# NilsJochem/audio-matcher

Hardware: AMD Instinct MI355X
Metric: audio samples/s matched (whole node), 10 s needle vs 1 h haystack, 1/2/4/8 GPU (higher is better)
Workload: dtype f32

## Files before the change

audio-matcher_amd/build.py:

```python
from __future__ import annotations

import os
import shutil
import subprocess
import sys
from concurrent.futures import ThreadPoolExecutor

HERE = os.path.dirname(os.path.abspath(__file__))
CSRC = os.path.join(HERE, "csrc")
OBJ = os.path.join(HERE, "build")
LIB = os.path.join(HERE, "libaudiomatch_amd.so")
SOURCES = ["am_fft.hip", "am_peaks.hip", "am_context.hip", "am_correlate.hip", "am_engine.hip", "am_stream.hip", "am_monitor.hip", "am_pool.hip", "am_norm.hip", "am_hits.hip", "am_segments.hip", "am_bands.hip", "am_significance.hip", "am_resample.hip", "am_whiten.hip", "am_estimate.hip", "am_warp.hip", "am_channel.hip", "am_stereo.hip",
           "am_best.hip", "am_trace.hip", "am_api.hip"]
HEADERS = [os.path.join(CSRC, "am_kernels.h"), os.path.join(CSRC, "am_internal.h"), os.path.join(CSRC, "am_walk.h"), os.path.join(CSRC, "am_spans.h"),
           os.path.join(HERE, "..", "include", "audiomatch.h")]
ARCH = "gfx950"
FLAGS = ["-O3", "-std=c++17", "-fPIC", f"--offload-arch={ARCH}", "-ffp-contract=fast", "-fno-slp-vectorize",
         "-Wall", "-Wno-unused-result"]


def _hipcc() -> str:
    for cand in (shutil.which("hipcc"), "/opt/rocm/bin/hipcc"):
        if cand and os.path.exists(cand):
            return cand
    raise RuntimeError("hipcc not found: the HIP extension cannot be built")


def _stale(target: str, deps: list[str]) -> bool:
    if not os.path.exists(target):
        return True
    t = os.path.getmtime(target)
    return any(os.path.getmtime(d) > t for d in deps if os.path.exists(d))


def build_library(force: bool = False, verbose: bool = False) -> str:
    srcs = [os.path.join(CSRC, s) for s in SOURCES]
    if not force and not _stale(LIB, srcs + HEADERS + [os.path.abspath(__file__)]):
# ... 82 lines not shown
```

audio-matcher_amd/csrc/am_fft.hip:

```cpp
#include "am_kernels.h"

#include <float.h>
#include <stdlib.h>
#include <algorithm>
#include <atomic>
#include <hip/hip_fp16.h>

namespace am {

__device__ __forceinline__ float2 cadd(float2 a, float2 b) { return make_float2(a.x + b.x, a.y + b.y); }
__device__ __forceinline__ float2 csub(float2 a, float2 b) { return make_float2(a.x - b.x, a.y - b.y); }
__device__ __forceinline__ float2 cmul(float2 a, float2 b) {
    return make_float2(a.x * b.x - a.y * b.y, a.x * b.y + a.y * b.x);
}
__device__ __forceinline__ float2 cmulc(float2 a, float2 b) {
    return make_float2(a.x * b.x + a.y * b.y, a.y * b.x - a.x * b.y);
}
__device__ __forceinline__ float2 mul_neg_i(float2 a) { return make_float2(a.y, -a.x); }
__device__ __forceinline__ float2 mul_pos_i(float2 a) { return make_float2(-a.y, a.x); }

__device__ __forceinline__ float2 tw_big(const PlanDev& pl, unsigned m) {
    return cmul(pl.twhi[m >> pl.logLo], pl.twlo[m & ((1u << pl.logLo) - 1u)]);
}

__device__ __forceinline__ void tw_big_pair(const PlanDev& pl, unsigned m, float2& w, float2& w4) {
    const float4 h = pl.twhi4[m >> pl.logLo], l = pl.twlo4[m & ((1u << pl.logLo) - 1u)];
    w = cmul(make_float2(h.x, h.y), make_float2(l.x, l.y));
    w4 = cmul(make_float2(h.z, h.w), make_float2(l.z, l.w));
}

__device__ constexpr float kCos32[16] = {
    1.0f, 0.9807852804032304f, 0.9238795325112867f, 0.8314696123025452f, 0.7071067811865476f,
    0.5555702330196023f, 0.38268343236508984f, 0.19509032201612833f, 0.0f, -0.1950903220161282f,
    -0.3826834323650897f, -0.555570233019602f, -0.7071067811865475f, -0.8314696123025453f,
    -0.9238795325112867f, -0.9807852804032304f};
__device__ constexpr float kSin32[16] = {
    0.0f, 0.19509032201612825f, 0.3826834323650898f, 0.5555702330196022f, 0.7071067811865475f,
    0.8314696123025452f, 0.9238795325112867f, 0.9807852804032304f, 1.0f, 0.9807852804032304f,
    0.9238795325112867f, 0.8314696123025455f, 0.7071067811865476f, 0.5555702330196022f,
    0.3826834323650899f, 0.1950903220161286f};

template <int R>
__host__ __device__ constexpr int brev(int i) {
    int r = 0;
    for (int b = 1; b < R; b <<= 1) { r = (r << 1) | (i & 1); i >>= 1; }
    return r;
}

template <bool INV>
__device__ __forceinline__ float2 mul_w32(float2 d, int idx) {
    if (idx == 0) return d;
    if (idx == 8) return INV ? mul_pos_i(d) : mul_neg_i(d);
    const float c = kCos32[idx], s = kSin32[idx];
    if (INV) return make_float2(d.x * c - d.y * s, d.x * s + d.y * c);
    return make_float2(d.x * c + d.y * s, d.y * c - d.x * s);
}

typedef _Float16 h2 __attribute__((ext_vector_type(2)));
__device__ __forceinline__ h2 cadd(h2 a, h2 b) { return a + b; }
__device__ __forceinline__ h2 csub(h2 a, h2 b) { return a - b; }
__device__ __forceinline__ h2 cmul(h2 a, h2 b) {
    const h2 t = a * b.xx;
    return __builtin_elementwise_fma(a.yx, (h2){-b.y, b.y}, t);
}
__device__ __forceinline__ h2 mul_neg_i(h2 a) { return (h2){a.y, -a.x}; }
__device__ __forceinline__ h2 mul_pos_i(h2 a) { return (h2){-a.y, a.x}; }
__device__ __forceinline__ h2 to_h2(float2 v) { return (h2){(_Float16)v.x, (_Float16)v.y}; }
__device__ __forceinline__ float2 to_f2(h2 v) { return make_float2((float)v.x, (float)v.y); }
__device__ __forceinline__ unsigned h2_bits(h2 v) { return __builtin_bit_cast(unsigned, v); }
__device__ __forceinline__ h2 bits_h2(unsigned u) { return __builtin_bit_cast(h2, u); }
template <bool INV>
__device__ __forceinline__ h2 mul_w32(h2 d, int idx) {
    if (idx == 0) return d;
    if (idx == 8) return INV ? mul_pos_i(d) : mul_neg_i(d);
    const _Float16 c = (_Float16)kCos32[idx], s = (_Float16)kSin32[idx];
    const h2 t = d * (h2){c, c};
    if (INV) return __builtin_elementwise_fma(d.yx, (h2){-s, s}, t);
    return __builtin_elementwise_fma(d.yx, (h2){s, -s}, t);
}

__device__ __forceinline__ float2 add_signed(float2 u, float2 v, float sgn) {
    return make_float2(fmaf(sgn, v.x, u.x), fmaf(sgn, v.y, u.y));
}

template <int R, bool INV, typename T>
__device__ __forceinline__ void dif(T* x) {
    if constexpr (R >= 2) {
#pragma unroll
        for (int i = 0; i < R / 2; ++i) {
            const T a = x[i], b = x[i + R / 2];
            x[i] = cadd(a, b);
            x[i + R / 2] = mul_w32<INV>(csub(a, b), i * (32 / R));
        }
        dif<R / 2, INV>(x);
        dif<R / 2, INV>(x + R / 2);
    }
}

template <int R, bool CONJ, bool BREV>
__device__ __forceinline__ void twiddle_apply(float2* x, float2 w) {
    float2 pw[R / 2 + 1];
    if (CONJ) w.y = -w.y;
    pw[1] = w;
    x[BREV ? brev<R>(1) : 1] = cmul(x[BREV ? brev<R>(1) : 1], w);
#pragma unroll
    for (int e = 2; e < R; ++e) {
        const float2 v = cmul(pw[(e + 1) / 2], pw[e / 2]);
        if (e <= R / 2) pw[e] = v;
        x[BREV ? brev<R>(e) : e] = cmul(x[BREV ? brev<R>(e) : e], v);
    }
}
template <int R, bool CONJ, bool BREV>
__device__ __forceinline__ void twiddle_apply(h2* x, float2 w) {
    float2 pw[R / 2 + 1];
    if (CONJ) w.y = -w.y;
    pw[1] = w;
    x[BREV ? brev<R>(1) : 1] = cmul(x[BREV ? brev<R>(1) : 1], to_h2(w));
#pragma unroll
    for (int e = 2; e < R; ++e) {
// ... 180 lines not shown
template <int KIND>
__device__ __forceinline__ void k1_load(const Job& job, long long col, int in_stride, int hi, long long baseA, long long baseB,
                                        bool validB, bool fast, float2 (&x0)[16], float2 (&x1)[16]) {
    if (fast) {
#pragma unroll
        for (int a = 0; a < 16; ++a) {
            const long long off = (long long)(a * 16 + hi) * in_stride + col;
            const float2 va = load_sample2<KIND>(job.src, baseA + off), vb = load_sample2<KIND>(job.src, baseB + off);
            x0[a] = make_float2(va.x, vb.x);
            x1[a] = make_float2(va.y, vb.y);
        }
    } else {
#pragma unroll
        for (int a = 0; a < 16; ++a) {
            const long long n = (long long)(a * 16 + hi) * in_stride + col;
            const float2 va = load2_padded<KIND>(job.src, baseA + n, job.src_len);
            const float2 vb = validB ? load2_padded<KIND>(job.src, baseB + n, job.src_len) : make_float2(0.f, 0.f);
            x0[a] = make_float2(va.x, vb.x);
            x1[a] = make_float2(va.y, vb.y);
        }
    }
}
__device__ __forceinline__ void k1_transform(const K1Twiddles& w, float2* lds2, int hi, int cp, float2 (&x0)[16], float2 (&x1)[16]) {
    dif<16, false>(x0);
    dif<16, false>(x1);
    twiddle_brev<16, false>(x0, w.w256, w.w256q);
    twiddle_brev<16, false>(x1, w.w256, w.w256q);
#pragma unroll
    for (int ap = 0; ap < 16; ++ap) lds2[(ap * 16 + hi) * 17 + cp] = x0[brev<16>(ap)];
    __syncthreads();
#pragma unroll
    for (int b = 0; b < 16; ++b) x0[b] = lds2[(hi * 16 + b) * 17 + cp];
    __syncthreads();
#pragma unroll
    for (int ap = 0; ap < 16; ++ap) lds2[(ap * 16 + hi) * 17 + cp] = x1[brev<16>(ap)];
    __syncthreads();
#pragma unroll
    for (int b = 0; b < 16; ++b) x1[b] = lds2[(hi * 16 + b) * 17 + cp];
    dif<16, false>(x0);
    dif<16, false>(x1);
    twiddle_chain<16, false, true>(x0, w.base0, w.step0, w.step0q);
    twiddle_chain<16, false, true>(x1, w.base1, w.step1, w.step1q);
}
template <int KIND>
__device__ __forceinline__ void k1_tile(const Job& job, const PlanDev& pl, float2* lds2, long long col, int in_stride,
                                        int hi, int cp, long long baseA, long long baseB, bool validB, bool fast,
                                        float2 (&x0)[16], float2 (&x1)[16]) {
    const K1Twiddles w = k1_twiddles(pl, col, hi);
    k1_load<KIND>(job, col, in_stride, hi, baseA, baseB, validB, fast, x0, x1);
    k1_transform(w, lds2, hi, cp, x0, x1);
}

__device__ __forceinline__ void k1_transform_h16(const K1Twiddles& w, uint2* ldsu, int hi, int cp, h2 (&x0)[16], h2 (&x1)[16]) {
    dif<16, false>(x0);
    dif<16, false>(x1);
    twiddle_apply2<16, false, true>(x0, x1, w.w256);
#pragma unroll
    for (int ap = 0; ap < 16; ++ap) ldsu[(ap * 16 + hi) * 17 + cp] = make_uint2(h2_bits(x0[brev<16>(ap)]), h2_bits(x1[brev<16>(ap)]));
    __syncthreads();
#pragma unroll
    for (int b = 0; b < 16; ++b) {
        const uint2 v = ldsu[(hi * 16 + b) * 17 + cp];
        x0[b] = bits_h2(v.x);
// ... 81 lines not shown
    float2 qj0, qj1, qc0, qc1;
};
__device__ __forceinline__ K2Lane k2_lane(const PlanDev& pl, int t = threadIdx.x) {
    K2Lane k;
    k.t = t; k.hi = k.t >> 4; k.cp = k.t & 15;
    k.voff = (unsigned)k.t * 16u;
    const float4 j = pl.k2j[2 * k.t], jq = pl.k2j[2 * k.t + 1], c = pl.k2c[2 * k.cp], cq = pl.k2c[2 * k.cp + 1];
    k.wj0 = make_float2(j.x, j.y); k.wj1 = make_float2(j.z, j.w);
    k.qj0 = make_float2(jq.x, jq.y); k.qj1 = make_float2(jq.z, jq.w);
    k.wc0 = make_float2(c.x, c.y); k.wc1 = make_float2(c.z, c.w);
    k.qc0 = make_float2(cq.x, cq.y); k.qc1 = make_float2(cq.z, cq.w);
    return k;
}

__device__ __forceinline__ void k2_forward12(const K2Lane& k, __amdgpu_buffer_rsrc_t rrow, float4* lds4) {
    const int t = k.t, hi = k.hi, cp = k.cp;
    float2 x0[16], x1[16];
#pragma unroll
    for (int a = 0; a < 16; ++a) {
        const float4 v = buf_load4(rrow, k.voff, a * 4096);
        x0[a] = make_float2(v.x, v.y);
        x1[a] = make_float2(v.z, v.w);
    }
    dif<16, false>(x0);
    dif<16, false>(x1);
    twiddle_brev<16, false>(x0, k.wj0, k.qj0);
    twiddle_brev<16, false>(x1, k.wj1, k.qj1);
#pragma unroll
    for (int ap = 0; ap < 16; ++ap)
        lds4[ap * 256 + t] = make_float4(x0[brev<16>(ap)].x, x0[brev<16>(ap)].y,
                                         x1[brev<16>(ap)].x, x1[brev<16>(ap)].y);
    __syncthreads();
#pragma unroll
    for (int b = 0; b < 16; ++b) {
        const float4 v = lds4[hi * 256 + b * 16 + cp];
        x0[b] = make_float2(v.x, v.y);
        x1[b] = make_float2(v.z, v.w);
    }
    dif<16, false>(x0);
    dif<16, false>(x1);
    twiddle_brev<16, false>(x0, k.wc0, k.qc0);
    twiddle_brev<16, false>(x1, k.wc1, k.qc1);
    wave_sync_lds();
#pragma unroll
    for (int bp = 0; bp < 16; ++bp)
        lds4[(hi * 16 + bp) * 16 + (cp ^ bp)] = make_float4(x0[brev<16>(bp)].x, x0[brev<16>(bp)].y,
                                                            x1[brev<16>(bp)].x, x1[brev<16>(bp)].y);
    wave_sync_lds();
}

__device__ __forceinline__ void k2_forward3(const K2Lane& k, const float4* lds4, float2 (&z)[32]) {
#pragma unroll
    for (int i = 0; i < 16; ++i) {
        const float4 v = lds4[k.t * 16 + (i ^ k.cp)];
        z[2 * i] = make_float2(v.x, v.y);
        z[2 * i + 1] = make_float2(v.z, v.w);
    }
    dif<32, false>(z);
}

__device__ __forceinline__ void k2_fetch_quarter(__amdgpu_buffer_rsrc_t rh, unsigned voff, int part, float4 (&h)[4]) {
#pragma unroll
    for (int i = 0; i < 4; ++i) h[i] = buf_load4(rh, voff, (part * 4 + i) * 4096);
}
__device__ __forceinline__ void k2_multiply_quarter(const float2 (&z)[32], const float4 (&h)[4], int part, float2 (&q)[32]) {
#pragma unroll
    for (int i = 0; i < 4; ++i) {
        const int e = part * 4 + i;
        q[brev<32>(2 * e)] = cmul(z[2 * e], make_float2(h[i].x, h[i].y));
        q[brev<32>(2 * e + 1)] = cmul(z[2 * e + 1], make_float2(h[i].z, h[i].w));
    }
}
__device__ __forceinline__ void k2_multiply_fetch(const float2 (&z)[32], __amdgpu_buffer_rsrc_t rh, unsigned voff,
                                                  const float4 (&first)[4], float2 (&q)[32]) {
    float4 ha[4], hb[4];
    k2_fetch_quarter(rh, voff, 1, ha);
    __builtin_amdgcn_sched_barrier(0);
    k2_multiply_quarter(z, first, 0, q);
    k2_fetch_quarter(rh, voff, 2, hb);
    __builtin_amdgcn_sched_barrier(0);
    k2_multiply_quarter(z, ha, 1, q);
// ... 142 lines not shown
__global__ void __launch_bounds__(256, kK2hWaves)
tail_rows_h16(unsigned* __restrict__ work, const unsigned* __restrict__ hc16, unsigned* __restrict__ dst, PlanDev pl, unsigned npairs,
              float pre) {
    k2_rows_h16_row(work, hc16, dst, pl, npairs, pre);
}

constexpr int kK2pWaves = 4;
template <bool HALF>
__device__ __forceinline__ void k2p_forward(const K2Lane& k, __amdgpu_buffer_rsrc_t rrow, float2* lds2, float2 (&z)[32]) {
    const int t = k.t, hi = k.hi, cp = k.cp;
    float2 x0[16], x1[16];
#pragma unroll
    for (int a = 0; a < 16; ++a) {
        if (HALF) {
            const uint2 v = buf_load_u2(rrow, k.voff / 2, a * 2048);
            x0[a] = unpack_h2(v.x);
            x1[a] = unpack_h2(v.y);
        } else {
            const float4 v = buf_load4(rrow, k.voff, a * 4096);
            x0[a] = make_float2(v.x, v.y);
            x1[a] = make_float2(v.z, v.w);
        }
    }
    dif<16, false>(x0);
    twiddle_brev<16, false>(x0, k.wj0, k.qj0);
#pragma unroll
    for (int ap = 0; ap < 16; ++ap) lds2[ap * kK2hSlab + t] = x0[brev<16>(ap)];
    dif<16, false>(x1);
    twiddle_brev<16, false>(x1, k.wj1, k.qj1);
    __syncthreads();
#pragma unroll
    for (int b = 0; b < 16; ++b) x0[b] = lds2[hi * kK2hSlab + b * 16 + cp];
    __syncthreads();
#pragma unroll
    for (int ap = 0; ap < 16; ++ap) lds2[ap * kK2hSlab + t] = x1[brev<16>(ap)];
    dif<16, false>(x0);
    twiddle_brev<16, false>(x0, k.wc0, k.qc0);
    __syncthreads();
#pragma unroll
    for (int b = 0; b < 16; ++b) x1[b] = lds2[hi * kK2hSlab + b * 16 + cp];
    wave_sync_lds();
#pragma unroll
    for (int bp = 0; bp < 16; ++bp) lds2[hi * kK2hSlab + bp * 16 + (cp ^ bp)] = x0[brev<16>(bp)];
    dif<16, false>(x1);
    twiddle_brev<16, false>(x1, k.wc1, k.qc1);
    wave_sync_lds();
#pragma unroll
    for (int i = 0; i < 16; ++i) z[2 * i] = lds2[hi * kK2hSlab + cp * 16 + (i ^ cp)];
    wave_sync_lds();
#pragma unroll
    for (int bp = 0; bp < 16; ++bp) lds2[hi * kK2hSlab + bp * 16 + (cp ^ bp)] = x1[brev<16>(bp)];
    wave_sync_lds();
#pragma unroll
    for (int i = 0; i < 16; ++i) z[2 * i + 1] = lds2[hi * kK2hSlab + cp * 16 + (i ^ cp)];
}

template <bool HALF, int SAUX = 0, bool LATE_J = false>
__device__ __forceinline__ void k2p_inverse(const PlanDev& pl, float2 (&q)[32], float2* lds2, __amdgpu_buffer_rsrc_t rdst) {
    int t = threadIdx.x;
    asm volatile("" : "+v"(t));
    const int hi = t >> 4, cp = t & 15;
    K2Lane ki;
    ki.t = t; ki.hi = hi; ki.cp = cp; ki.voff = (unsigned)t * 16u;
    {
        const float4 c = pl.k2c[2 * cp], cq = pl.k2c[2 * cp + 1];
        ki.wc0 = make_float2(c.x, c.y); ki.wc1 = make_float2(c.z, c.w);
        ki.qc0 = make_float2(cq.x, cq.y); ki.qc1 = make_float2(cq.z, cq.w);
    }
    if (!LATE_J) {
        const float4 j = pl.k2j[2 * t], jq = pl.k2j[2 * t + 1];
        ki.wj0 = make_float2(j.x, j.y); ki.wj1 = make_float2(j.z, j.w);
        ki.qj0 = make_float2(jq.x, jq.y); ki.qj1 = make_float2(jq.z, jq.w);
    }
    const K2Lane& k = ki;
    float2 x0[16], x1[16];
    dif<32, true>(q);
    wave_sync_lds();
#pragma unroll
    for (int i = 0; i < 16; ++i) lds2[hi * kK2hSlab + cp * 16 + (i ^ cp)] = q[brev<32>(2 * i)];
    wave_sync_lds();
#pragma unroll
    for (int bp = 0; bp < 16; ++bp) x0[bp] = lds2[hi * kK2hSlab + bp * 16 + (cp ^ bp)];
    wave_sync_lds();
#pragma unroll
    for (int i = 0; i < 16; ++i) lds2[hi * kK2hSlab + cp * 16 + (i ^ cp)] = q[brev<32>(2 * i + 1)];
    twiddle_nat<16, true>(x0, ki.wc0, ki.qc0);
    dif<16, true>(x0);
    wave_sync_lds();
#pragma unroll
    for (int bp = 0; bp < 16; ++bp) x1[bp] = lds2[hi * kK2hSlab + bp * 16 + (cp ^ bp)];
    wave_sync_lds();
#pragma unroll
    for (int b = 0; b < 16; ++b) lds2[hi * kK2hSlab + b * 16 + cp] = x0[brev<16>(b)];
    if (LATE_J) {
        __builtin_amdgcn_sched_barrier(0);
        const float4 j = pl.k2j[2 * t], jq = pl.k2j[2 * t + 1];
        ki.wj0 = make_float2(j.x, j.y); ki.wj1 = make_float2(j.z, j.w);
        ki.qj0 = make_float2(jq.x, jq.y); ki.qj1 = make_float2(jq.z, jq.w);
        __builtin_amdgcn_sched_barrier(0);
    }
    twiddle_nat<16, true>(x1, ki.wc1, ki.qc1);
    dif<16, true>(x1);
    __syncthreads();
#pragma unroll
    for (int ap = 0; ap < 16; ++ap) x0[ap] = lds2[ap * kK2hSlab + t];
    __syncthreads();
#pragma unroll
    for (int b = 0; b < 16; ++b) lds2[hi * kK2hSlab + b * 16 + cp] = x1[brev<16>(b)];
    twiddle_nat<16, true>(x0, ki.wj0, ki.qj0);
    dif<16, true>(x0);
    __syncthreads();
#pragma unroll
    for (int ap = 0; ap < 16; ++ap) x1[ap] = lds2[ap * kK2hSlab + t];
    twiddle_nat<16, true>(x1, ki.wj1, ki.qj1);
    dif<16, true>(x1);
    if (HALF) {
#pragma unroll
        for (int a = 0; a < 16; ++a)
            buf_store_u2(rdst, k.voff / 2, a * 2048, make_uint2(pack_h2(x0[brev<16>(a)]), pack_h2(x1[brev<16>(a)])));
        return;
    }
#pragma unroll
    for (int a = 0; a < 16; ++a)
        buf_store4<SAUX>(rdst, k.voff, a * 4096, make_float4(x0[brev<16>(a)].x, x0[brev<16>(a)].y,
                                                           x1[brev<16>(a)].x, x1[brev<16>(a)].y));
}

template <bool HALF>
__device__ __forceinline__ void k2_rows_r16_planes_row(float2* __restrict__ work, const float2* __restrict__ hc, float2* __restrict__ dst,
                                                       const PlanDev& pl, unsigned npairs, float hscale) {
    extern __shared__ float4 lds4[];
    float2* lds2 = reinterpret_cast<float2*>(lds4);
    unsigned row, slot;
    k2_place(npairs, row, slot);
    const size_t row_off = ((size_t)slot << pl.logN) + (size_t)row * kN2;
    const __amdgpu_buffer_rsrc_t rrow = HALF ? make_rsrc(reinterpret_cast<unsigned*>(work) + row_off, kN2 * 4)
                                             : make_rsrc(work + row_off, kN2 * 8);
    const __amdgpu_buffer_rsrc_t rdst = !dst ? rrow
        : HALF ? make_rsrc(reinterpret_cast<unsigned*>(dst) + row_off, kN2 * 4) : make_rsrc(dst + row_off, kN2 * 8);
    const __amdgpu_buffer_rsrc_t rh = make_rsrc(reinterpret_cast<const float4*>(hc) + (size_t)row * (kN2 / 2), kN2 * 8);
    const K2Lane k = k2_lane(pl);
    float2 z[32];
    k2p_forward<HALF>(k, rrow, lds2, z);
    float4 ha[4], hb[4], hc4[4];
    __builtin_amdgcn_sched_barrier(0);
    k2_fetch_quarter(rh, k.voff, 0, ha);
    k2_fetch_quarter(rh, k.voff, 1, hb);
    __builtin_amdgcn_sched_barrier(0);
    dif<32, false>(z);
    __builtin_amdgcn_sched_barrier(0);
    k2_fetch_quarter(rh, k.voff, 2, hc4);
    __builtin_amdgcn_sched_barrier(0);
    auto scaled = [&](float4 (&h)[4]) {
        if (HALF) {
#pragma unroll
            for (int i = 0; i < 4; ++i) { h[i].x *= hscale; h[i].y *= hscale; h[i].z *= hscale; h[i].w *= hscale; }
        }
    };
    float2 q[32];
    scaled(ha);
    k2_multiply_quarter(z, ha, 0, q);
    k2_fetch_quarter(rh, k.voff, 3, ha);
    __builtin_amdgcn_sched_barrier(0);
    scaled(hb);
    k2_multiply_quarter(z, hb, 1, q);
    scaled(hc4);
    k2_multiply_quarter(z, hc4, 2, q);
    scaled(ha);
    k2_multiply_quarter(z, ha, 3, q);
    k2p_inverse<HALF>(pl, q, lds2, rdst);
}
template <bool HALF>
// ... 3 lines not shown
    k2_rows_r16_planes_row<HALF>(work, hc, dst, pl, npairs, hscale);
}
template <bool HALF>
__global__ void __launch_bounds__(256, kK2pWaves)
tail_rows_r16_planes(float2* __restrict__ work, const float2* __restrict__ hc, float2* __restrict__ dst, PlanDev pl, unsigned npairs,
                     float hscale) {
    k2_rows_r16_planes_row<HALF>(work, hc, dst, pl, npairs, hscale);
}

constexpr int kK2gpWaves = 3;
constexpr int kK2gStoreAux = 2;
__global__ void __launch_bounds__(256, kK2gpWaves)
k2_rows_r16_group_planes(const float2* __restrict__ work, K2Group grp, PlanDev pl, unsigned npairs) {
    extern __shared__ float4 lds4[];
    float2* lds2 = reinterpret_cast<float2*>(lds4);
    unsigned row, slot;
    k2_place(npairs, row, slot);
    const size_t row_off = ((size_t)slot << pl.logN) + (size_t)row * kN2;
    const __amdgpu_buffer_rsrc_t rrow = make_rsrc(work + row_off, kN2 * 8);
    const size_t hoff4 = (size_t)row * (kN2 / 2);
    const K2Lane k = k2_lane(pl);
    float2 z[32];
    k2p_forward<false>(k, rrow, lds2, z);
    dif<32, false>(z);
#pragma unroll 1
    for (int j = 0; j < grp.n; ++j) {
        const __amdgpu_buffer_rsrc_t rh = make_rsrc(reinterpret_cast<const float4*>(grp.hc[j]) + hoff4, kN2 * 8);
        float4 hq[4];
        k2_fetch_quarter(rh, k.voff, 0, hq);
        float2 q[32];
        k2_multiply_fetch(z, rh, k.voff, hq, q);
        k2p_inverse<false, kK2gStoreAux, true>(pl, q, lds2, make_rsrc(grp.dst[j] + row_off, kN2 * 8));
        __syncthreads();
    }
}

__global__ void __launch_bounds__(256) spectrum_to_half_kernel(const float2* __restrict__ hc, long long n, float scale, unsigned* __restrict__ out) {
    for (long long i = (long long)blockIdx.x * 256 + threadIdx.x; i < n; i += (long long)gridDim.x * 256)
        out[i] = h2_bits(to_h2(make_float2(hc[i].x * scale, hc[i].y * scale)));
}
hipError_t launch_spectrum_to_half(hipStream_t st, const float2* hc, long long n, float scale, unsigned* out) {
    hipLaunchKernelGGL(spectrum_to_half_kernel, dim3(2048), dim3(256), 0, st, hc, n, scale, out);
    return hipGetLastError();
}

typedef _Float16 half8 __attribute__((ext_vector_type(8)));
typedef float f32x4v __attribute__((ext_vector_type(4)));
// ... 453 lines not shown
}


template <bool ACC = false>
__device__ __forceinline__ void k3_tile(const Job& job, const PlanDev& pl, const ScanCfg& scan, float2* lds2,
                                        int n2_0, int out_stride, int t, long long blkA, long long blkB,
                                        float out_scale, float2 (&x0)[16], float2 (&x1)[16], const ScanCfg* geo = nullptr) {
    const int hi = t >> 4, cp = t & 15;
    const long long N = 1ll << pl.logN;
    const long long col = n2_0 + 2 * cp;
    const K3Edges ed = k3_edges(job, geo ? *geo : scan, blkA, blkB);
    const unsigned maskN = (unsigned)(N - 1);
    const float2 w256 = pl.tw1[hi], w256q = pl.tw1[4 * hi];
    {
        const unsigned n2 = (unsigned)col;
        float2 base0 = tw_big(pl, (n2 * (unsigned)hi) & maskN);
        float2 base1 = tw_big(pl, ((n2 + 1) * (unsigned)hi) & maskN);
        base0.x *= out_scale; base0.y *= out_scale;
        base1.x *= out_scale; base1.y *= out_scale;
        float2 step0, step1, step0q, step1q;
        tw_big_pair(pl, (n2 * 16u) & maskN, step0, step0q);
        tw_big_pair(pl, ((n2 + 1) * 16u) & maskN, step1, step1q);
        twiddle_chain<16, true, false>(x0, base0, step0, step0q);
        dif<16, true>(x0);
#pragma unroll
        for (int b = 0; b < 16; ++b) lds2[(hi * 16 + b) * 16 + cp] = x0[brev<16>(b)];
        twiddle_chain<16, true, false>(x1, base1, step1, step1q);
    }
    dif<16, true>(x1);
    __syncthreads();
#pragma unroll
    for (int ap = 0; ap < 16; ++ap) x0[ap] = lds2[(ap * 16 + hi) * 16 + cp];
    __syncthreads();
#pragma unroll
    for (int b = 0; b < 16; ++b) lds2[(hi * 16 + b) * 16 + cp] = x1[brev<16>(b)];
    twiddle_nat<16, true>(x0, w256, w256q);
    dif<16, true>(x0);
    __syncthreads();
#pragma unroll
    for (int ap = 0; ap < 16; ++ap) x1[ap] = lds2[(ap * 16 + hi) * 16 + cp];
    twiddle_nat<16, true>(x1, w256, w256q);
    dif<16, true>(x1);
    k3_finish<4, ACC, true>(job, scan, ed, lds2, n2_0, out_stride, t, blkA, blkB, out_scale, x0, x1);
}

__device__ __forceinline__ void k3_tile_h16(const Job& job, const PlanDev& pl, const ScanCfg& scan, float2* lds2,
                                            int n2_0, int out_stride, int t, long long blkA, long long blkB,
                                            float out_scale, h2 (&hx0)[16], h2 (&hx1)[16]) {
    const int hi = t >> 4, cp = t & 15;
    const long long N = 1ll << pl.logN;
    const long long col = n2_0 + 2 * cp;
    const K3Edges ed = k3_edges(job, scan, blkA, blkB);
    const unsigned maskN = (unsigned)(N - 1);
    const float2 w256 = pl.tw1[hi];
    {
        const unsigned n2 = (unsigned)col;
        const float2 base0 = tw_big(pl, (n2 * (unsigned)hi) & maskN);
        const float2 base1 = tw_big(pl, ((n2 + 1) * (unsigned)hi) & maskN);
        const float2 step0 = tw_big(pl, (n2 * 16u) & maskN);
        const float2 step1 = tw_big(pl, ((n2 + 1) * 16u) & maskN);
        twiddle_chain<16, true, false>(hx0, base0, step0);
        twiddle_chain<16, true, false>(hx1, base1, step1);
    }
    dif<16, true>(hx0);
    dif<16, true>(hx1);
// ... 233 lines not shown
    twiddle_brev<16, false>(x1, w512, w512q);
    float2 y0[16], y1[16];
#pragma unroll
    for (int a2 = 0; a2 < 16; ++a2) lds2[c512_idx(a2, hi, cp)] = x0[brev<16>(a2)];
    __syncthreads();
#pragma unroll
    for (int b = 0; b < 16; ++b) {
        const float2 lo = lds2[c512_idx(ap, b, cp)], up = lds2[c512_idx(ap, b + 16, cp)];
        y0[b] = half ? mul_w32<false>(csub(lo, up), b) : cadd(lo, up);
    }
    __syncthreads();
#pragma unroll
    for (int a2 = 0; a2 < 16; ++a2) lds2[c512_idx(a2, hi, cp)] = x1[brev<16>(a2)];
    __syncthreads();
#pragma unroll
    for (int b = 0; b < 16; ++b) {
        const float2 lo = lds2[c512_idx(ap, b, cp)], up = lds2[c512_idx(ap, b + 16, cp)];
        y1[b] = half ? mul_w32<false>(csub(lo, up), b) : cadd(lo, up);
    }
    __builtin_amdgcn_sched_barrier(0);
    tw_big_pair(pl, ((unsigned)col * 32u) & maskN, step0, step0q);
    tw_big_pair(pl, (((unsigned)col + 1u) * 32u) & maskN, step1, step1q);
    __builtin_amdgcn_sched_barrier(0);
    dif<16, false>(y0);
    dif<16, false>(y1);
    twiddle_chain<16, false, true>(y0, base0, step0, step0q);
    twiddle_chain<16, false, true>(y1, base1, step1, step1q);
    if (HALF) {
        uint2* __restrict__ out2 = reinterpret_cast<uint2*>(reinterpret_cast<unsigned*>(work) + ((size_t)blockIdx.y << pl.logN) + n2_0) + cp;
#pragma unroll
        for (int bt = 0; bt < 16; ++bt) {
            const size_t k1 = (size_t)(k10 + 32 * bt);
            out2[k1 * (kN2 / 2)] = make_uint2(pack_h2(y0[brev<16>(bt)]), pack_h2(y1[brev<16>(bt)]));
        }
        return;
    }
    float4* __restrict__ out4 = reinterpret_cast<float4*>(work + ((size_t)blockIdx.y << pl.logN) + n2_0) + cp;
#pragma unroll
    for (int bt = 0; bt < 16; ++bt) {
        const size_t k1 = (size_t)(k10 + 32 * bt);
        out4[k1 * (kN2 / 2)] = make_float4(y0[brev<16>(bt)].x, y0[brev<16>(bt)].y,
                                             y1[brev<16>(bt)].x, y1[brev<16>(bt)].y);
    }
}

template <int HALF, bool ACC, int LN2 = kR16LogN2>
__device__ __forceinline__ void k3_cols_inv_c512_tile(unsigned lin, float4* lds4, const Job& job, const float2* __restrict__ work,
                                                      const PlanDev& pl, float out_scale, const ScanCfg& scan, const ScanCfg* geo = nullptr) {
// ... 74 lines not shown
            x1[bt] = unpack_h2(v.y);
        }
    } else {
        const __amdgpu_buffer_rsrc_t rin = make_rsrc(work + ((size_t)slot << pl.logN) + n2_0, (unsigned)((N - n2_0) * 8));
        const unsigned voff = (unsigned)k10 * (kN2 * 8u) + (unsigned)cp * 16u;
#pragma unroll
        for (int bt = 0; bt < 16; ++bt) {
            const float4 v = buf_load4<kK3LoadAux>(rin, voff, (unsigned)bt * (32u * kN2 * 8u));
            x0[bt] = make_float2(v.x, v.y);
            x1[bt] = make_float2(v.z, v.w);
        }
    }
    const K3Edges ed = k3_edges(job, geo ? *geo : scan, blkA, blkB);
    const float2 w512 = pl.tw1[hi], w512q = pl.tw1[4 * hi];
    {
        float2 base0 = tw_big(pl, (n2 * (unsigned)k10) & maskN);
        float2 base1 = tw_big(pl, ((n2 + 1u) * (unsigned)k10) & maskN);
        base0.x *= out_scale; base0.y *= out_scale;
        base1.x *= out_scale; base1.y *= out_scale;
        float2 step0, step1, step0q, step1q;
        tw_big_pair(pl, (n2 * 32u) & maskN, step0, step0q);
        tw_big_pair(pl, ((n2 + 1u) * 32u) & maskN, step1, step1q);
        twiddle_chain<16, true, false>(x0, base0, step0, step0q);
        dif<16, true>(x0);
        if (half) {
#pragma unroll
            for (int b = 1; b < 16; ++b) x0[brev<16>(b)] = mul_w32<true>(x0[brev<16>(b)], b);
        }
#pragma unroll
        for (int b = 0; b < 16; ++b) lds2[c512_idx3(ap, b + 16 * half, cp)] = x0[brev<16>(b)];
        twiddle_chain<16, true, false>(x1, base1, step1, step1q);
    }
    dif<16, true>(x1);
    if (half) {
#pragma unroll
        for (int b = 1; b < 16; ++b) x1[brev<16>(b)] = mul_w32<true>(x1[brev<16>(b)], b);
    }
    const float sgn = hi >= 16 ? -1.0f : 1.0f;
    const int bb = hi & 15;
    __syncthreads();
#pragma unroll
    for (int a2 = 0; a2 < 16; ++a2) {
        const float2 u = lds2[c512_idx3(a2, bb, cp)], v = lds2[c512_idx3(a2, bb + 16, cp)];
        x0[a2] = add_signed(u, v, sgn);
    }
    __syncthreads();
#pragma unroll
    for (int b = 0; b < 16; ++b) lds2[c512_idx3(ap, b + 16 * half, cp)] = x1[brev<16>(b)];
    twiddle_nat<16, true>(x0, w512, w512q);
    dif<16, true>(x0);
    __syncthreads();
#pragma unroll
    for (int a2 = 0; a2 < 16; ++a2) {
        const float2 u = lds2[c512_idx3(a2, bb, cp)], v = lds2[c512_idx3(a2, bb + 16, cp)];
        x1[a2] = add_signed(u, v, sgn);
    }
    twiddle_nat<16, true>(x1, w512, w512q);
    dif<16, true>(x1);
    k3_finish<5, ACC, true>(job, scan, ed, lds2, n2_0, kN2, t, blkA, blkB, out_scale, x0, x1);
}
template <int HALF, bool ACC = false, int REDO = 0>
__global__ void __launch_bounds__(512, REDO ? 4 : 2)
k3_cols_inv_c512(Job job, const float2* __restrict__ work, PlanDev pl, float out_scale, ScanCfg scan) {
    extern __shared__ float4 lds4[];
    if constexpr (REDO != 0) {
        for (unsigned lin = blockIdx.x; lin < (unsigned)scan.redo_tiles; lin += gridDim.x) {
            k3_cols_inv_c512_tile<HALF, ACC>(lin, lds4, job, work, pl, out_scale, scan);
            __syncthreads();
        }
    } else {
        k3_cols_inv_c512_tile<HALF, ACC>(blockIdx.x, lds4, job, work, pl, out_scale, scan);
    }
}

__global__ void __launch_bounds__(512, 2)
k3_cols_inv_c512w(Job job, const float2* __restrict__ work, PlanDev pl, float out_scale, ScanCfg scan) {
    extern __shared__ float4 lds4[];
    k3_cols_inv_c512_tile<0, false, 14>(blockIdx.x, lds4, job, work, pl, out_scale, scan);
}

__global__ void __launch_bounds__(512, 2)
// ... 632 lines not shown
```

Baseline: 228.8 billion.

## Replace DIF radix-16/32 butterflies with FMA-based DIT and fused twiddle stages

Moves the complex helpers into a shared header and adds a decimation-in-time butterfly built on FMAs, where b = 2a - (a + w*b). Most dif<16>/dif<32> calls in the FFT kernels become dit. In the inverse column passes, the separate twiddle_nat multiply followed by a DIF is merged into dit_tw, which folds the per-element twiddles into the first butterfly stage. The goal is fewer VALU instructions per butterfly, at the cost of slightly different rounding from the 2a-p formulation and reliance on the DIT output order matching the old DIF bit-reversed order.

```diff
diff --git a/audio-matcher_amd/build.py b/audio-matcher_amd/build.py
--- a/audio-matcher_amd/build.py
+++ b/audio-matcher_amd/build.py
@@ -12,7 +12,7 @@
 LIB = os.path.join(HERE, "libaudiomatch_amd.so")
 SOURCES = ["am_fft.hip", "am_peaks.hip", "am_context.hip", "am_correlate.hip", "am_engine.hip", "am_stream.hip", "am_monitor.hip", "am_pool.hip", "am_norm.hip", "am_hits.hip", "am_segments.hip", "am_bands.hip", "am_significance.hip", "am_resample.hip", "am_whiten.hip", "am_estimate.hip", "am_warp.hip", "am_channel.hip", "am_stereo.hip",
            "am_best.hip", "am_trace.hip", "am_api.hip"]
-HEADERS = [os.path.join(CSRC, "am_kernels.h"), os.path.join(CSRC, "am_internal.h"), os.path.join(CSRC, "am_walk.h"), os.path.join(CSRC, "am_spans.h"),
+HEADERS = [os.path.join(CSRC, "am_kernels.h"), os.path.join(CSRC, "am_internal.h"), os.path.join(CSRC, "am_walk.h"), os.path.join(CSRC, "am_spans.h"), os.path.join(CSRC, "am_butterfly.h"),
            os.path.join(HERE, "..", "include", "audiomatch.h")]
 ARCH = "gfx950"
 FLAGS = ["-O3", "-std=c++17", "-fPIC", f"--offload-arch={ARCH}", "-ffp-contract=fast", "-fno-slp-vectorize",
diff --git a/audio-matcher_amd/csrc/am_butterfly.h b/audio-matcher_amd/csrc/am_butterfly.h
--- /dev/null
+++ b/audio-matcher_amd/csrc/am_butterfly.h
@@ -0,0 +1,186 @@
+#pragma once
+
+#if defined(__HIPCC__)
+#include <hip/hip_runtime.h>
+#define AM_HD __host__ __device__ __forceinline__
+#define AM_TABLE __device__ constexpr
+#else
+#define AM_HD inline
+#define AM_TABLE constexpr
+struct float2 { float x, y; };
+inline float2 make_float2(float x, float y) { float2 v; v.x = x; v.y = y; return v; }
+#endif
+
+namespace am {
+
+AM_HD float2 cadd(float2 a, float2 b) { return make_float2(a.x + b.x, a.y + b.y); }
+AM_HD float2 csub(float2 a, float2 b) { return make_float2(a.x - b.x, a.y - b.y); }
+AM_HD float2 cmul(float2 a, float2 b) {
+    return make_float2(a.x * b.x - a.y * b.y, a.x * b.y + a.y * b.x);
+}
+AM_HD float2 cmulc(float2 a, float2 b) {
+    return make_float2(a.x * b.x + a.y * b.y, a.y * b.x - a.x * b.y);
+}
+AM_HD float2 mul_neg_i(float2 a) { return make_float2(a.y, -a.x); }
+AM_HD float2 mul_pos_i(float2 a) { return make_float2(-a.y, a.x); }
+
+AM_TABLE float kCos32[16] = {
+    1.0f, 0.9807852804032304f, 0.9238795325112867f, 0.8314696123025452f, 0.7071067811865476f,
+    0.5555702330196023f, 0.38268343236508984f, 0.19509032201612833f, 0.0f, -0.1950903220161282f,
+    -0.3826834323650897f, -0.555570233019602f, -0.7071067811865475f, -0.8314696123025453f,
+    -0.9238795325112867f, -0.9807852804032304f};
+AM_TABLE float kSin32[16] = {
+    0.0f, 0.19509032201612825f, 0.3826834323650898f, 0.5555702330196022f, 0.7071067811865475f,
+    0.8314696123025452f, 0.9238795325112867f, 0.9807852804032304f, 1.0f, 0.9807852804032304f,
+    0.9238795325112867f, 0.8314696123025455f, 0.7071067811865476f, 0.5555702330196022f,
+    0.3826834323650899f, 0.1950903220161286f};
+
+template <int R>
+AM_HD constexpr int brev(int i) {
+    int r = 0;
+    for (int b = 1; b < R; b <<= 1) { r = (r << 1) | (i & 1); i >>= 1; }
+    return r;
+}
+
+template <bool INV>
+AM_HD float2 mul_w32(float2 d, int idx) {
+    if (idx == 0) return d;
+    if (idx == 8) return INV ? mul_pos_i(d) : mul_neg_i(d);
+    const float c = kCos32[idx], s = kSin32[idx];
+    if (INV) return make_float2(d.x * c - d.y * s, d.x * s + d.y * c);
+    return make_float2(d.x * c + d.y * s, d.y * c - d.x * s);
+}
+
+#if defined(__HIPCC__)
+typedef _Float16 h2 __attribute__((ext_vector_type(2)));
+__device__ __forceinline__ h2 cadd(h2 a, h2 b) { return a + b; }
+__device__ __forceinline__ h2 csub(h2 a, h2 b) { return a - b; }
+__device__ __forceinline__ h2 cmul(h2 a, h2 b) {
+    const h2 t = a * b.xx;
+    return __builtin_elementwise_fma(a.yx, (h2){-b.y, b.y}, t);
+}
+__device__ __forceinline__ h2 mul_neg_i(h2 a) { return (h2){a.y, -a.x}; }
+__device__ __forceinline__ h2 mul_pos_i(h2 a) { return (h2){-a.y, a.x}; }
+__device__ __forceinline__ h2 to_h2(float2 v) { return (h2){(_Float16)v.x, (_Float16)v.y}; }
+__device__ __forceinline__ float2 to_f2(h2 v) { return make_float2((float)v.x, (float)v.y); }
+__device__ __forceinline__ unsigned h2_bits(h2 v) { return __builtin_bit_cast(unsigned, v); }
+__device__ __forceinline__ h2 bits_h2(unsigned u) { return __builtin_bit_cast(h2, u); }
+template <bool INV>
+__device__ __forceinline__ h2 mul_w32(h2 d, int idx) {
+    if (idx == 0) return d;
+    if (idx == 8) return INV ? mul_pos_i(d) : mul_neg_i(d);
+    const _Float16 c = (_Float16)kCos32[idx], s = (_Float16)kSin32[idx];
+    const h2 t = d * (h2){c, c};
+    if (INV) return __builtin_elementwise_fma(d.yx, (h2){-s, s}, t);
+    return __builtin_elementwise_fma(d.yx, (h2){s, -s}, t);
+}
+#endif
+
+template <int R, bool INV, typename T>
+AM_HD void dif(T* x) {
+    if constexpr (R >= 2) {
+#pragma unroll
+        for (int i = 0; i < R / 2; ++i) {
+            const T a = x[i], b = x[i + R / 2];
+            x[i] = cadd(a, b);
+            x[i + R / 2] = mul_w32<INV>(csub(a, b), i * (32 / R));
+        }
+        dif<R / 2, INV>(x);
+        dif<R / 2, INV>(x + R / 2);
+    }
+}
+
+template <bool INV>
+AM_HD void dit_bfly(float2& a, float2& b, int idx) {
+    if (idx == 0) {
+        const float2 p = cadd(a, b);
+        b = csub(a, b);
+        a = p;
+        return;
+    }
+    if (idx == 8) {
+        const float2 t = INV ? mul_pos_i(b) : mul_neg_i(b);
+        b = csub(a, t);
+        a = cadd(a, t);
+        return;
+    }
+    const float c = kCos32[idx], s = INV ? kSin32[idx] : -kSin32[idx];
+    float2 p;
+    p.x = __builtin_fmaf(b.y, -s, __builtin_fmaf(b.x, c, a.x));
+    p.y = __builtin_fmaf(b.x, s, __builtin_fmaf(b.y, c, a.y));
+    b = make_float2(__builtin_fmaf(2.0f, a.x, -p.x), __builtin_fmaf(2.0f, a.y, -p.y));
+    a = p;
+}
+
+template <int R, int M, bool INV>
+AM_HD void dit_stage(float2* x) {
+    constexpr int S = R / M;
+#pragma unroll
+    for (int o = 0; o < S; ++o) {
+#pragma unroll
+        for (int k = 0; k < M / 2; ++k) {
+            const int ia = o + 2 * brev<M / 2>(k) * S;
+            dit_bfly<INV>(x[ia], x[ia + S], k * (32 / M));
+        }
+    }
+}
+template <int R, bool INV, int M = 2>
+AM_HD void dit(float2* x) {
+    if constexpr (M <= R) {
+        dit_stage<R, M, INV>(x);
+        dit<R, INV, 2 * M>(x);
+    }
+}
+
+AM_HD void dit_bfly_tw(float2& a, float2& b, float2 ta, float2 tb) {
+    const float2 u = cmul(a, ta);
+    float2 p;
+    p.x = __builtin_fmaf(-b.y, tb.y, __builtin_fmaf(b.x, tb.x, u.x));
+    p.y = __builtin_fmaf(b.x, tb.y, __builtin_fmaf(b.y, tb.x, u.y));
+    b = make_float2(__builtin_fmaf(2.0f, u.x, -p.x), __builtin_fmaf(2.0f, u.y, -p.y));
+    a = p;
+}
+AM_HD void dit_bfly_tw(float2& a, float2& b, float2 tb) {
+    float2 p;
+    p.x = __builtin_fmaf(-b.y, tb.y, __builtin_fmaf(b.x, tb.x, a.x));
+    p.y = __builtin_fmaf(b.x, tb.y, __builtin_fmaf(b.y, tb.x, a.y));
+    b = make_float2(__builtin_fmaf(2.0f, a.x, -p.x), __builtin_fmaf(2.0f, a.y, -p.y));
+    a = p;
+}
+
+template <int R, bool INV>
+AM_HD void dit_tw(float2* x, float2 w, float2 w4) {
+    static_assert(R == 16, "powers 1..15 from w and w^4");
+    if (INV) { w.y = -w.y; w4.y = -w4.y; }
+    float2 pw[R];
+    pw[1] = w; pw[2] = cmul(w, w); pw[3] = cmul(pw[2], w);
+    float2 g = w4;
+#pragma unroll
+    for (int e = 4; e < R; ++e) {
+        if ((e & 3) == 0 && e > 4) g = cmul(g, w4);
+        pw[e] = (e & 3) == 0 ? g : cmul(g, pw[e & 3]);
+    }
+    dit_bfly_tw(x[0], x[R / 2], pw[R / 2]);
+#pragma unroll
+    for (int e = 1; e < R / 2; ++e) dit_bfly_tw(x[e], x[e + R / 2], pw[e], pw[e + R / 2]);
+    dit<R, INV, 4>(x);
+}
+template <int R, bool INV>
+AM_HD void dit_tw(float2* x, float2 base, float2 step, float2 step4) {
+    static_assert(R == 16, "four runs of four");
+    if (INV) { base.y = -base.y; step.y = -step.y; step4.y = -step4.y; }
+    float2 pw[R];
+    float2 g = base;
+#pragma unroll
+    for (int k = 0; k < R; k += 4) {
+        if (k) g = cmul(g, step4);
+        pw[k] = g;
+#pragma unroll
+        for (int j = 1; j < 4; ++j) pw[k + j] = cmul(pw[k + j - 1], step);
+    }
+#pragma unroll
+    for (int e = 0; e < R / 2; ++e) dit_bfly_tw(x[e], x[e + R / 2], pw[e], pw[e + R / 2]);
+    dit<R, INV, 4>(x);
+}
+
+}
diff --git a/audio-matcher_amd/csrc/am_fft.hip b/audio-matcher_amd/csrc/am_fft.hip
--- a/audio-matcher_amd/csrc/am_fft.hip
+++ b/audio-matcher_amd/csrc/am_fft.hip
@@ -1,4 +1,5 @@
 #include "am_kernels.h"
+#include "am_butterfly.h"
 
 #include <float.h>
 #include <stdlib.h>
@@ -8,17 +9,6 @@
 
 namespace am {
 
-__device__ __forceinline__ float2 cadd(float2 a, float2 b) { return make_float2(a.x + b.x, a.y + b.y); }
-__device__ __forceinline__ float2 csub(float2 a, float2 b) { return make_float2(a.x - b.x, a.y - b.y); }
-__device__ __forceinline__ float2 cmul(float2 a, float2 b) {
-    return make_float2(a.x * b.x - a.y * b.y, a.x * b.y + a.y * b.x);
-}
-__device__ __forceinline__ float2 cmulc(float2 a, float2 b) {
-    return make_float2(a.x * b.x + a.y * b.y, a.y * b.x - a.x * b.y);
-}
-__device__ __forceinline__ float2 mul_neg_i(float2 a) { return make_float2(a.y, -a.x); }
-__device__ __forceinline__ float2 mul_pos_i(float2 a) { return make_float2(-a.y, a.x); }
-
 __device__ __forceinline__ float2 tw_big(const PlanDev& pl, unsigned m) {
     return cmul(pl.twhi[m >> pl.logLo], pl.twlo[m & ((1u << pl.logLo) - 1u)]);
 }
@@ -29,72 +19,8 @@
     w4 = cmul(make_float2(h.z, h.w), make_float2(l.z, l.w));
 }
 
-__device__ constexpr float kCos32[16] = {
-    1.0f, 0.9807852804032304f, 0.9238795325112867f, 0.8314696123025452f, 0.7071067811865476f,
-    0.5555702330196023f, 0.38268343236508984f, 0.19509032201612833f, 0.0f, -0.1950903220161282f,
-    -0.3826834323650897f, -0.555570233019602f, -0.7071067811865475f, -0.8314696123025453f,
-    -0.9238795325112867f, -0.9807852804032304f};
-__device__ constexpr float kSin32[16] = {
-    0.0f, 0.19509032201612825f, 0.3826834323650898f, 0.5555702330196022f, 0.7071067811865475f,
-    0.8314696123025452f, 0.9238795325112867f, 0.9807852804032304f, 1.0f, 0.9807852804032304f,
-    0.9238795325112867f, 0.8314696123025455f, 0.7071067811865476f, 0.5555702330196022f,
-    0.3826834323650899f, 0.1950903220161286f};
-
-template <int R>
-__host__ __device__ constexpr int brev(int i) {
-    int r = 0;
-    for (int b = 1; b < R; b <<= 1) { r = (r << 1) | (i & 1); i >>= 1; }
-    return r;
-}
-
-template <bool INV>
-__device__ __forceinline__ float2 mul_w32(float2 d, int idx) {
-    if (idx == 0) return d;
-    if (idx == 8) return INV ? mul_pos_i(d) : mul_neg_i(d);
-    const float c = kCos32[idx], s = kSin32[idx];
-    if (INV) return make_float2(d.x * c - d.y * s, d.x * s + d.y * c);
-    return make_float2(d.x * c + d.y * s, d.y * c - d.x * s);
-}
-
-typedef _Float16 h2 __attribute__((ext_vector_type(2)));
-__device__ __forceinline__ h2 cadd(h2 a, h2 b) { return a + b; }
-__device__ __forceinline__ h2 csub(h2 a, h2 b) { return a - b; }
-__device__ __forceinline__ h2 cmul(h2 a, h2 b) {
-    const h2 t = a * b.xx;
-    return __builtin_elementwise_fma(a.yx, (h2){-b.y, b.y}, t);
-}
-__device__ __forceinline__ h2 mul_neg_i(h2 a) { return (h2){a.y, -a.x}; }
-__device__ __forceinline__ h2 mul_pos_i(h2 a) { return (h2){-a.y, a.x}; }
-__device__ __forceinline__ h2 to_h2(float2 v) { return (h2){(_Float16)v.x, (_Float16)v.y}; }
-__device__ __forceinline__ float2 to_f2(h2 v) { return make_float2((float)v.x, (float)v.y); }
-__device__ __forceinline__ unsigned h2_bits(h2 v) { return __builtin_bit_cast(unsigned, v); }
-__device__ __forceinline__ h2 bits_h2(unsigned u) { return __builtin_bit_cast(h2, u); }
-template <bool INV>
-__device__ __forceinline__ h2 mul_w32(h2 d, int idx) {
-    if (idx == 0) return d;
-    if (idx == 8) return INV ? mul_pos_i(d) : mul_neg_i(d);
-    const _Float16 c = (_Float16)kCos32[idx], s = (_Float16)kSin32[idx];
-    const h2 t = d * (h2){c, c};
-    if (INV) return __builtin_elementwise_fma(d.yx, (h2){-s, s}, t);
-    return __builtin_elementwise_fma(d.yx, (h2){s, -s}, t);
-}
-
 __device__ __forceinline__ float2 add_signed(float2 u, float2 v, float sgn) {
     return make_float2(fmaf(sgn, v.x, u.x), fmaf(sgn, v.y, u.y));
-}
-
-template <int R, bool INV, typename T>
-__device__ __forceinline__ void dif(T* x) {
-    if constexpr (R >= 2) {
-#pragma unroll
-        for (int i = 0; i < R / 2; ++i) {
-            const T a = x[i], b = x[i + R / 2];
-            x[i] = cadd(a, b);
-            x[i + R / 2] = mul_w32<INV>(csub(a, b), i * (32 / R));
-        }
-        dif<R / 2, INV>(x);
-        dif<R / 2, INV>(x + R / 2);
-    }
 }
 
 template <int R, bool CONJ, bool BREV>
@@ -321,8 +247,8 @@
     }
 }
 __device__ __forceinline__ void k1_transform(const K1Twiddles& w, float2* lds2, int hi, int cp, float2 (&x0)[16], float2 (&x1)[16]) {
-    dif<16, false>(x0);
-    dif<16, false>(x1);
+    dit<16, false>(x0);
+    dit<16, false>(x1);
     twiddle_brev<16, false>(x0, w.w256, w.w256q);
     twiddle_brev<16, false>(x1, w.w256, w.w256q);
 #pragma unroll
@@ -336,8 +262,8 @@
     __syncthreads();
 #pragma unroll
     for (int b = 0; b < 16; ++b) x1[b] = lds2[(hi * 16 + b) * 17 + cp];
-    dif<16, false>(x0);
-    dif<16, false>(x1);
+    dit<16, false>(x0);
+    dit<16, false>(x1);
     twiddle_chain<16, false, true>(x0, w.base0, w.step0, w.step0q);
     twiddle_chain<16, false, true>(x1, w.base1, w.step1, w.step1q);
 }
@@ -465,8 +391,8 @@
         x0[a] = make_float2(v.x, v.y);
         x1[a] = make_float2(v.z, v.w);
     }
-    dif<16, false>(x0);
-    dif<16, false>(x1);
+    dit<16, false>(x0);
+    dit<16, false>(x1);
     twiddle_brev<16, false>(x0, k.wj0, k.qj0);
     twiddle_brev<16, false>(x1, k.wj1, k.qj1);
 #pragma unroll
@@ -480,8 +406,8 @@
         x0[b] = make_float2(v.x, v.y);
         x1[b] = make_float2(v.z, v.w);
     }
-    dif<16, false>(x0);
-    dif<16, false>(x1);
+    dit<16, false>(x0);
+    dit<16, false>(x1);
     twiddle_brev<16, false>(x0, k.wc0, k.qc0);
     twiddle_brev<16, false>(x1, k.wc1, k.qc1);
     wave_sync_lds();
@@ -499,7 +425,7 @@
         z[2 * i] = make_float2(v.x, v.y);
         z[2 * i + 1] = make_float2(v.z, v.w);
     }
-    dif<32, false>(z);
+    dit<32, false>(z);
 }
 
 __device__ __forceinline__ void k2_fetch_quarter(__amdgpu_buffer_rsrc_t rh, unsigned voff, int part, float4 (&h)[4]) {
@@ -688,11 +614,11 @@
             x1[a] = make_float2(v.z, v.w);
         }
     }
-    dif<16, false>(x0);
+    dit<16, false>(x0);
     twiddle_brev<16, false>(x0, k.wj0, k.qj0);
 #pragma unroll
     for (int ap = 0; ap < 16; ++ap) lds2[ap * kK2hSlab + t] = x0[brev<16>(ap)];
-    dif<16, false>(x1);
+    dit<16, false>(x1);
     twiddle_brev<16, false>(x1, k.wj1, k.qj1);
     __syncthreads();
 #pragma unroll
@@ -700,7 +626,7 @@
     __syncthreads();
 #pragma unroll
     for (int ap = 0; ap < 16; ++ap) lds2[ap * kK2hSlab + t] = x1[brev<16>(ap)];
-    dif<16, false>(x0);
+    dit<16, false>(x0);
     twiddle_brev<16, false>(x0, k.wc0, k.qc0);
     __syncthreads();
 #pragma unroll
@@ -708,7 +634,7 @@
     wave_sync_lds();
 #pragma unroll
     for (int bp = 0; bp < 16; ++bp) lds2[hi * kK2hSlab + bp * 16 + (cp ^ bp)] = x0[brev<16>(bp)];
-    dif<16, false>(x1);
+    dit<16, false>(x1);
     twiddle_brev<16, false>(x1, k.wc1, k.qc1);
     wave_sync_lds();
 #pragma unroll
@@ -740,7 +666,7 @@
     }
     const K2Lane& k = ki;
     float2 x0[16], x1[16];
-    dif<32, true>(q);
+    dit<32, true>(q);
     wave_sync_lds();
 #pragma unroll
     for (int i = 0; i < 16; ++i) lds2[hi * kK2hSlab + cp * 16 + (i ^ cp)] = q[brev<32>(2 * i)];
@@ -750,8 +676,7 @@
     wave_sync_lds();
 #pragma unroll
     for (int i = 0; i < 16; ++i) lds2[hi * kK2hSlab + cp * 16 + (i ^ cp)] = q[brev<32>(2 * i + 1)];
-    twiddle_nat<16, true>(x0, ki.wc0, ki.qc0);
-    dif<16, true>(x0);
+    dit_tw<16, true>(x0, ki.wc0, ki.qc0);
     wave_sync_lds();
 #pragma unroll
     for (int bp = 0; bp < 16; ++bp) x1[bp] = lds2[hi * kK2hSlab + bp * 16 + (cp ^ bp)];
@@ -765,21 +690,18 @@
         ki.qj0 = make_float2(jq.x, jq.y); ki.qj1 = make_float2(jq.z, jq.w);
         __builtin_amdgcn_sched_barrier(0);
     }
-    twiddle_nat<16, true>(x1, ki.wc1, ki.qc1);
-    dif<16, true>(x1);
+    dit_tw<16, true>(x1, ki.wc1, ki.qc1);
     __syncthreads();
 #pragma unroll
     for (int ap = 0; ap < 16; ++ap) x0[ap] = lds2[ap * kK2hSlab + t];
     __syncthreads();
 #pragma unroll
     for (int b = 0; b < 16; ++b) lds2[hi * kK2hSlab + b * 16 + cp] = x1[brev<16>(b)];
-    twiddle_nat<16, true>(x0, ki.wj0, ki.qj0);
-    dif<16, true>(x0);
+    dit_tw<16, true>(x0, ki.wj0, ki.qj0);
     __syncthreads();
 #pragma unroll
     for (int ap = 0; ap < 16; ++ap) x1[ap] = lds2[ap * kK2hSlab + t];
-    twiddle_nat<16, true>(x1, ki.wj1, ki.qj1);
-    dif<16, true>(x1);
+    dit_tw<16, true>(x1, ki.wj1, ki.qj1);
     if (HALF) {
 #pragma unroll
         for (int a = 0; a < 16; ++a)
@@ -813,7 +735,7 @@
     k2_fetch_quarter(rh, k.voff, 0, ha);
     k2_fetch_quarter(rh, k.voff, 1, hb);
     __builtin_amdgcn_sched_barrier(0);
-    dif<32, false>(z);
+    dit<32, false>(z);
     __builtin_amdgcn_sched_barrier(0);
     k2_fetch_quarter(rh, k.voff, 2, hc4);
     __builtin_amdgcn_sched_barrier(0);
@@ -863,7 +785,7 @@
     const K2Lane k = k2_lane(pl);
     float2 z[32];
     k2p_forward<false>(k, rrow, lds2, z);
-    dif<32, false>(z);
+    dit<32, false>(z);
 #pragma unroll 1
     for (int j = 0; j < grp.n; ++j) {
         const __amdgpu_buffer_rsrc_t rh = make_rsrc(reinterpret_cast<const float4*>(grp.hc[j]) + hoff4, kN2 * 8);
@@ -1363,25 +1285,23 @@
         tw_big_pair(pl, (n2 * 16u) & maskN, step0, step0q);
         tw_big_pair(pl, ((n2 + 1) * 16u) & maskN, step1, step1q);
         twiddle_chain<16, true, false>(x0, base0, step0, step0q);
-        dif<16, true>(x0);
+        dit<16, true>(x0);
 #pragma unroll
         for (int b = 0; b < 16; ++b) lds2[(hi * 16 + b) * 16 + cp] = x0[brev<16>(b)];
         twiddle_chain<16, true, false>(x1, base1, step1, step1q);
-    }
-    dif<16, true>(x1);
+        dit<16, true>(x1);
+    }
     __syncthreads();
 #pragma unroll
     for (int ap = 0; ap < 16; ++ap) x0[ap] = lds2[(ap * 16 + hi) * 16 + cp];
     __syncthreads();
 #pragma unroll
     for (int b = 0; b < 16; ++b) lds2[(hi * 16 + b) * 16 + cp] = x1[brev<16>(b)];
-    twiddle_nat<16, true>(x0, w256, w256q);
-    dif<16, true>(x0);
+    dit_tw<16, true>(x0, w256, w256q);
     __syncthreads();
 #pragma unroll
     for (int ap = 0; ap < 16; ++ap) x1[ap] = lds2[(ap * 16 + hi) * 16 + cp];
-    twiddle_nat<16, true>(x1, w256, w256q);
-    dif<16, true>(x1);
+    dit_tw<16, true>(x1, w256, w256q);
     k3_finish<4, ACC, true>(job, scan, ed, lds2, n2_0, out_stride, t, blkA, blkB, out_scale, x0, x1);
 }
 
@@ -1661,8 +1581,8 @@
     tw_big_pair(pl, ((unsigned)col * 32u) & maskN, step0, step0q);
     tw_big_pair(pl, (((unsigned)col + 1u) * 32u) & maskN, step1, step1q);
     __builtin_amdgcn_sched_barrier(0);
-    dif<16, false>(y0);
-    dif<16, false>(y1);
+    dit<16, false>(y0);
+    dit<16, false>(y1);
     twiddle_chain<16, false, true>(y0, base0, step0, step0q);
     twiddle_chain<16, false, true>(y1, base1, step1, step1q);
     if (HALF) {
@@ -1783,7 +1703,7 @@
         tw_big_pair(pl, (n2 * 32u) & maskN, step0, step0q);
         tw_big_pair(pl, ((n2 + 1u) * 32u) & maskN, step1, step1q);
         twiddle_chain<16, true, false>(x0, base0, step0, step0q);
-        dif<16, true>(x0);
+        dit<16, true>(x0);
         if (half) {
 #pragma unroll
             for (int b = 1; b < 16; ++b) x0[brev<16>(b)] = mul_w32<true>(x0[brev<16>(b)], b);
@@ -1791,8 +1711,8 @@
 #pragma unroll
         for (int b = 0; b < 16; ++b) lds2[c512_idx3(ap, b + 16 * half, cp)] = x0[brev<16>(b)];
         twiddle_chain<16, true, false>(x1, base1, step1, step1q);
-    }
-    dif<16, true>(x1);
+        dit<16, true>(x1);
+    }
     if (half) {
 #pragma unroll
         for (int b = 1; b < 16; ++b) x1[brev<16>(b)] = mul_w32<true>(x1[brev<16>(b)], b);
@@ -1808,16 +1728,14 @@
     __syncthreads();
 #pragma unroll
     for (int b = 0; b < 16; ++b) lds2[c512_idx3(ap, b + 16 * half, cp)] = x1[brev<16>(b)];
-    twiddle_nat<16, true>(x0, w512, w512q);
-    dif<16, true>(x0);
+    dit_tw<16, true>(x0, w512, w512q);
     __syncthreads();
 #pragma unroll
     for (int a2 = 0; a2 < 16; ++a2) {
         const float2 u = lds2[c512_idx3(a2, bb, cp)], v = lds2[c512_idx3(a2, bb + 16, cp)];
         x1[a2] = add_signed(u, v, sgn);
     }
-    twiddle_nat<16, true>(x1, w512, w512q);
-    dif<16, true>(x1);
+    dit_tw<16, true>(x1, w512, w512q);
     k3_finish<5, ACC, true>(job, scan, ed, lds2, n2_0, kN2, t, blkA, blkB, out_scale, x0, x1);
 }
 template <int HALF, bool ACC = false, int REDO = 0>
```

Result: no change. 228.6 billion, median of 2 (-0.1%).
